# carrenD/Medical-Cross-Modality-Domain-Adaptation

Measured on AMD Instinct MI355X. Metric: training slices/sec (256x256x3, B=16/GPU) joint segmenter+GAN step (1 dis update on B MR + B CT, clip, 1 gen update on B CT), higher is better.
Workload: dtype f32; 1 GPU; BASELINE configs[3]: train_gan.py --phase train-gan joint step, B=16/GPU per domain, f32, dropout .75, mask critic on; global_batch=16, per_gpu_batch=16, parallelism=dp1, step_capture=False

## Files before the change

medical-cross-modality-domain-adaptation_amd/csrc/conv_common.h:

```cpp
#pragma once
#include "pnp_common.h"

namespace pnpconv {

constexpr int BK = 32;
constexpr int NTHREADS = 256;
#ifndef PNP_CONV_ABLATE
#define PNP_CONV_ABLATE 0
#endif
constexpr int kAblate = PNP_CONV_ABLATE;

struct ConvArgs {
    const float* x;
    const float* w;
    float* y;
    int N, H, W, C, K, R, S, OH, OW, stride, dil, pad_t, pad_l, pad_mode;
    int ups;
    int M;
    int Kred;
    int OHW;
    int nblk_m, nblk_n;
    int gn;
    int nsplit, chunks_per_split;
    long long split_stride;
// ... 302 lines not shown
int launch_x3_direct(const ConvArgs& a, int kind, bool flip_transpose, void* ws, size_t ws_bytes, hipStream_t st);
bool wino_chosen(const pnp_conv_geom* g);
int wino_tile(const pnp_conv_geom* g);
size_t wino_workspace_bytes(const pnp_conv_geom* g);
int wino_stats_parts(const pnp_conv_geom* g);
int launch_wino(const ConvArgs& a, int kind, bool flip_transpose, void* ws, size_t ws_bytes, hipStream_t st);
bool wino_wgrad_chosen(const pnp_conv_geom* g);
int wino_wgrad_tile(const pnp_conv_geom* g);
size_t wino_wgrad_workspace_bytes(const pnp_conv_geom* g);
int launch_wino_wgrad(const ConvArgs& a, float* dw, int accumulate, void* ws, size_t ws_bytes, hipStream_t st);
#ifndef PNP_X3_SW
#define PNP_X3_SW 32
#endif
constexpr int X3_SW = PNP_X3_SW;
static_assert(X3_SW == 16 || X3_SW == 32, "stage width");
bool wino_x3_dims_ok(int T, int C, int K);
int launch_wino_gemm_x3(const unsigned short* V3, const unsigned short* U3, float* Mm, int T, int C, int K, int npos, int sym, int gn, int xcd,
                        int nsplit, int stages_per_split, hipStream_t st);
inline double conv_flops(const ConvArgs& a) { return 2.0 * (double)a.M * a.K * a.Kred; }
inline double conv_bytes(const ConvArgs& a) {
    return 4.0 * ((double)a.N * a.H * a.W * a.C + (double)a.M * a.K + (double)a.Kred * a.K);
}
inline int prof_class(int kind) { return kind == 0 ? PNP_PROF_CONV_FWD : PNP_PROF_CONV_DGRAD; }

}
```

medical-cross-modality-domain-adaptation_amd/csrc/conv_wino.hip:

```cpp
#include <atomic>
#include <map>
#include <mutex>
#include "conv_common.h"
#include "conv_mma.h"

using namespace pnpconv;

namespace {

constexpr int NT = 256;

__device__ __forceinline__ f32x4 ld4(const float* p) { return *reinterpret_cast<const f32x4*>(p); }
__device__ __forceinline__ void st4(float* p, f32x4 v) { *reinterpret_cast<f32x4*>(p) = v; }

typedef __bf16 bf16x4 __attribute__((ext_vector_type(4)));
__device__ __forceinline__ void split3(float v, __bf16& hi, __bf16& mid, __bf16& lo) {
    hi = (__bf16)v;
    const float r = v - (float)hi;
    mid = (__bf16)r;
    lo = (__bf16)(r - (float)mid);
}
__device__ __forceinline__ void st4x3(__bf16* p, size_t pstride, f32x4 v) {
    bf16x4 h, m, l;
#pragma unroll
    for (int e = 0; e < 4; ++e) {
        __bf16 a, b, c;
        split3(v[e], a, b, c);
        h[e] = a; m[e] = b; l[e] = c;
    }
    *reinterpret_cast<bf16x4*>(p) = h;
    *reinterpret_cast<bf16x4*>(p + pstride) = m;
    *reinterpret_cast<bf16x4*>(p + 2 * pstride) = l;
}

struct WinoGeom {
    int N, Hi, Wi, Ho, Wo, dil, ps, Hsi, Wsi, Hso, Wso, th, tw, T;
    int m;
};

template <typename V>
__device__ __forceinline__ void w4_bt(const V& d0, const V& d1, const V& d2, const V& d3, const V& d4, const V& d5, V* o) {
    o[0] = (d0 + d4) + (1.5f * (d3 - d1) - 2.f * d2);
    o[1] = (d4 - d1) + (0.5f * d2 + 2.5f * d3);
    o[2] = (d4 + d1) + (0.5f * d3 - 2.5f * d2);
    o[3] = (d4 - d2) + 2.f * (d3 - d1);
    o[4] = (d4 - d2) + 0.5f * (d1 - d3);
    o[5] = (d1 + d5) + (1.5f * (d4 - d2) - 2.f * d3);
}
// ... 69 lines not shown
        f32x4 d[P][P];
#pragma unroll
        for (int p = 0; p < P; ++p) {
            const int u = M * ti - a.g.ps + p;
            const bool uok = (unsigned)u < (unsigned)a.g.Hsi;
#pragma unroll
            for (int q = 0; q < P; ++q) {
                const int v = M * tj - a.g.ps + q;
                const bool ok = uok & ((unsigned)v < (unsigned)a.g.Wsi);
                const unsigned off = (unsigned)(((n * a.g.Hi + pa + a.g.dil * u) * a.g.Wi + pb + a.g.dil * v) * a.C + c) * 4u;
                d[p][q] = bload4(rx, ok ? off : OOB);
            }
        }
        f32x4 r[P][P];
        float* out = a.V + (size_t)t * a.C + c;
        __bf16* out3 = reinterpret_cast<__bf16*>(a.V) + ((size_t)(c / X3_SW) * 3 * a.g.T + t) * X3_SW + (c % X3_SW);
        auto put = [&](int pos, f32x4 v) {
            if constexpr (X3) st4x3(out3 + (size_t)pos * 3 * plane, (size_t)a.g.T * X3_SW, v);
            else st4(out + (size_t)pos * plane, v);
        };
        if constexpr (M == 2) {
#pragma unroll
            for (int q = 0; q < 4; ++q) {
                r[0][q] = d[0][q] - d[2][q];
                r[1][q] = d[1][q] + d[2][q];
                r[2][q] = d[2][q] - d[1][q];
                r[3][q] = d[1][q] - d[3][q];
            }
#pragma unroll
            for (int p = 0; p < 4; ++p) {
                put(4 * p + 0, r[p][0] - r[p][2]);
                put(4 * p + 1, r[p][1] + r[p][2]);
                put(4 * p + 2, r[p][2] - r[p][1]);
                put(4 * p + 3, r[p][1] - r[p][3]);
            }
// ... 568 lines not shown
            f32x4 c6[6];
            w4_a(y[0][q], y[1][q], y[2][q], y[3][q], c6);
#pragma unroll
            for (int p = 0; p < 6; ++p) z[p][q] = c6[p];
        }
#pragma unroll
        for (int p = 0; p < 6; ++p) {
            f32x4 o[6];
            w4_a(z[p][0], z[p][1], z[p][2], z[p][3], o);
#pragma unroll
            for (int q = 0; q < 6; ++q) v[6 * p + q] = o[q];
        }
    }
}
template <int NP, int PG>
__device__ __forceinline__ void emit_t(const f32x4 (&v)[NP], float (*tile)[32][34], __bf16* __restrict__ out, size_t pos_stride, int tblk, int rows, int ch0,
                                       int tid) {
    const int c4 = tid & 7, tl = tid >> 3;
    const int cl = tid >> 3, tq = tid & 7;
#pragma unroll
    for (int r0 = 0; r0 < NP; r0 += PG) {
#pragma unroll
        for (int p = 0; p < PG; ++p)
#pragma unroll
            for (int e = 0; e < 4; ++e) tile[p][c4 * 4 + e][tl] = v[r0 + p][e];
        __syncthreads();
        if (ch0 + cl < rows) {
#pragma unroll
            for (int p = 0; p < PG; ++p) {
                const float* src = &tile[p][cl][4 * tq];
                const f32x4 w = {src[0], src[1], src[2], src[3]};
                const int tg = tblk * 32 + 4 * tq;
                st4x3(out + (size_t)(r0 + p) * pos_stride + ((size_t)(tg / X3_SW) * 3 * rows + ch0 + cl) * X3_SW + (tg % X3_SW), (size_t)rows * X3_SW, w);
            }
        }
        __syncthreads();
    }
}
struct WinoTArgs {
    const float* src;
    __bf16* out;
    WinoGeom g;
    int rows;
    unsigned src_bytes;
    int ntb;
};
template <int M>
__global__ void __launch_bounds__(NT) wino_in_t_kernel(WinoTArgs a) {
    constexpr int P = M + 2, NP = P * P, PG = M == 4 ? 12 : 8;
    __shared__ float tile[PG][32][34];
    const int tid = threadIdx.x, c4 = tid & 7, tl = tid >> 3;
    const int t = blockIdx.x * 32 + tl, c = blockIdx.y * 32 + c4 * 4;
    const bool tok = t < a.g.T;
    const __amdgpu_buffer_rsrc_t rx = make_rsrc(a.src, a.src_bytes);
    int n, pa, pb, ti, tj;
    tile_of(a.g, tok ? t : 0, n, pa, pb, ti, tj);
    f32x4 d[P][P];
#pragma unroll
    for (int p = 0; p < P; ++p) {
        const int u = M * ti - a.g.ps + p;
        const bool uok = tok & ((unsigned)u < (unsigned)a.g.Hsi);
#pragma unroll
        for (int q = 0; q < P; ++q) {
            const int v_ = M * tj - a.g.ps + q;
            const bool ok = uok & ((unsigned)v_ < (unsigned)a.g.Wsi);
            const unsigned off = (unsigned)(((n * a.g.Hi + pa + a.g.dil * u) * a.g.Wi + pb + a.g.dil * v_) * a.rows + c) * 4u;
            d[p][q] = bload4(rx, ok ? off : OOB);
        }
    }
    f32x4 v[NP];
    bt_2d<M>(d, v);
    emit_t<NP, PG>(v, tile, a.out, (size_t)a.ntb * 3 * a.rows * 32, (int)blockIdx.x, a.rows, (int)blockIdx.y * 32, tid);
}
template <int M>
__global__ void __launch_bounds__(NT) wino_dy_t_kernel(WinoTArgs a) {
    constexpr int P = M + 2, NP = P * P, PG = M == 4 ? 12 : 8;
    __shared__ float tile[PG][32][34];
    const int tid = threadIdx.x, c4 = tid & 7, tl = tid >> 3;
    const int t = blockIdx.x * 32 + tl, k = blockIdx.y * 32 + c4 * 4;
    const bool tok = t < a.g.T && k < a.rows;
    int n, pa, pb, ti, tj;
    tile_of(a.g, t < a.g.T ? t : 0, n, pa, pb, ti, tj);
    f32x4 y[M][M];
#pragma unroll
    for (int p = 0; p < M; ++p)
#pragma unroll
        for (int q = 0; q < M; ++q) {
            const int u = M * ti + p, v_ = M * tj + q;
            const f32x4 zero = {0, 0, 0, 0};
            y[p][q] = (tok && u < a.g.Hso && v_ < a.g.Wso) ? ld4(a.src + ((size_t)(n * a.g.Ho + pa + a.g.dil * u) * a.g.Wo + pb + a.g.dil * v_) * a.rows + k) : zero;
        }
    f32x4 v[NP];
    a_2d<M>(y, v);
    emit_t<NP, PG>(v, tile, a.out, (size_t)a.ntb * 3 * a.rows * 32, (int)blockIdx.x, a.rows, (int)blockIdx.y * 32, tid);
}

struct WinoWgradGemmArgs {
    const float* V;
    const float* Y;
    float* S;
    int T, C, K;
    int nblk_m, nblk_n, nsplit, chunks_per_split, xcd_swizzle;
    int npos;
};

template <int BM, int BN, int WM, int WN, int TILE>
__global__ void __launch_bounds__(NTHREADS, 2) wino_wgrad_gemm_kernel(WinoWgradGemmArgs g) {
    constexpr int TM = BM / WM / 32, TN = BN / WN / 32;
    constexpr int LDA = BM + 4, LDB = BN + 4;
// ... 379 lines not shown

int wino_stats_parts(const pnp_conv_geom* g) {
    if (x3d_chosen(g)) return x3d_stats_parts(g);
    const int m = plan_tile(g, false);
    const WinoGeom w = make_wgeom(g, m ? m : 2);
    int tpb, nblk;
    out_plan(w.T, g->K, &tpb, &nblk);
    return nblk;
}

template <int M>
static int launch_wino_m(const ConvArgs& a, int kind, bool flip_transpose, void* ws, size_t ws_bytes, hipStream_t st) {
    constexpr int NP = (M + 2) * (M + 2);
    const WinoGeom w = make_wgeom(a.N, a.H, a.W, a.OH, a.OW, a.dil, a.pad_t, M);
    const bool x3 = use_x3(w.T, a.C, a.K);
    const size_t eb = x3 ? 6 : 4;
    const size_t ub = al256((size_t)NP * a.C * a.K * eb), vb = al256((size_t)NP * w.T * a.C * eb), mb = al256((size_t)NP * w.T * a.K * 4);
    static const int xcd_mode = env_int("PNP_WINO_XCD", 2);
    const bool xcd = a.xcd_swizzle && xcd_mode;
    GemmPlan plan = gemm_plan(w.T, a.C, a.K, NP, xcd);
    if (x3) { plan.s = 1; plan.px_bytes = 0; }
    if (!ws || ws_bytes < ub + vb + mb + plan.px_bytes) {
        pnp_set_error("launch_wino: workspace too small (%zu < %zu)", ws_bytes, ub + vb + mb + plan.px_bytes);
        return PNP_EWORKSPACE;
    }
    PNP_REQUIRE(a.y_h == nullptr && a.o_s == 0 && a.ups == 1, "launch_wino: unsupported epilogue");
    bool run_filter;
    float* U = filter_slot(a.w, flip_transpose ? 1 : 0, M, a.C, a.K, x3 ? 1 : 0, (size_t)NP * a.C * a.K * eb, (float*)ws, st, &run_filter);
    float* V = (float*)((char*)ws + ub);
    float* Mm = (float*)((char*)ws + ub + vb);
    float* Px = (float*)((char*)ws + ub + vb + mb);
// ... 2 lines not shown
        dim3 grid((unsigned)pnp_cdiv(a.K, 32), (unsigned)pnp_cdiv(a.C, 32));
        PnpProfScope ps(cls, st, 0.0, (36.0 + eb * NP) * a.C * a.K, "wino_filter_kernel<%s, %d, %s>", flip_transpose ? "true" : "false", M, x3 ? "true" : "false");
        if (x3) {
            if (flip_transpose) hipLaunchKernelGGL((wino_filter_kernel<true, M, true>), grid, dim3(NT), 0, st, a.w, U, a.C, a.K);
            else hipLaunchKernelGGL((wino_filter_kernel<false, M, true>), grid, dim3(NT), 0, st, a.w, U, a.C, a.K);
        } else if (flip_transpose) hipLaunchKernelGGL((wino_filter_kernel<true, M, false>), grid, dim3(NT), 0, st, a.w, U, a.C, a.K);
        else hipLaunchKernelGGL((wino_filter_kernel<false, M, false>), grid, dim3(NT), 0, st, a.w, U, a.C, a.K);
        PNP_CHECK_LAUNCH("wino_filter_kernel");
    }
    {
        WinoInArgs ia{};
        ia.x = a.x; ia.V = V; ia.g = w; ia.C = a.C; ia.x_bytes = a.x_bytes; ia.xcd = a.xcd_swizzle ? env_xcd_in() : 0;
        const size_t nvec = (size_t)w.T * (a.C / 4);
        long long nb = (long long)((nvec + NT - 1) / NT);
        if (nb > 65536) nb = 65536;
        PnpProfScope ps(cls, st, 0.0, 4.0 * (double)a.N * a.H * a.W * a.C + (double)eb * NP * w.T * a.C, "wino_in_kernel<%d, %s>", M, x3 ? "true" : "false");
        if (x3) hipLaunchKernelGGL((wino_in_kernel<M, true>), dim3((unsigned)nb), dim3(NT), 0, st, ia);
        else hipLaunchKernelGGL((wino_in_kernel<M, false>), dim3((unsigned)nb), dim3(NT), 0, st, ia);
        PNP_CHECK_LAUNCH("wino_in_kernel");
    }
    if (x3) {
        static const int wino_gn3 = env_int("PNP_WINO_GN", -1);
        const int rc = launch_wino_gemm_x3((const unsigned short*)V, (const unsigned short*)U, Mm, w.T, a.C, a.K, NP, (M == 4 ? 2 : 0) + (kind != 0), wino_gn3 >= 0 ? wino_gn3 : a.gn,
                                           xcd ? 1 : 0, 1, a.C / 32, st);
        if (rc != PNP_OK) return rc;
    } else {
        WinoGemmArgs ga{};
        ga.V = V; ga.U = U; ga.Mm = Mm; ga.T = w.T; ga.C = a.C; ga.K = a.K;
        const bool narrow = a.K <= 64;
        ga.nblk_m = pnp_cdiv(w.T, 128); ga.nblk_n = pnp_cdiv(a.K, narrow ? 64 : 128);
        static const int wino_gn = env_int("PNP_WINO_GN", -1);
        ga.gn = wino_gn >= 0 ? wino_gn : a.gn; ga.xcd_swizzle = xcd ? 2 : 0;
        ga.npos = NP;
        ga.whole = ((double)NP * w.T * a.C * 4.0 < 2147483648.0 && (double)NP * a.C * a.K * 4.0 < 2147483648.0) ? 1 : 0;
        ga.tail_F = plan.F; ga.tail_R = plan.R; ga.tail_s = plan.s; ga.Px = Px;
        dim3 grid((unsigned)plan.grid);
        const double fl = 2.0 * NP * (double)w.T * a.C * a.K;
        const double by = 4.0 * NP * ((double)w.T * a.C + (double)a.C * a.K + (double)w.T * a.K);
// ... 81 lines not shown
}

template <int M>
static int launch_wino_wgrad_m(const ConvArgs& a, float* dw, int accumulate, void* ws, size_t ws_bytes, hipStream_t st) {
    constexpr int NP = (M + 2) * (M + 2);
    const WinoGeom w = make_wgeom(a.N, a.H, a.W, a.OH, a.OW, a.dil, a.pad_t, M);
    if (use_x3_wgrad(w.T, a.C, a.K)) {
        int sps;
        const int ns = wgrad_split_x3(w.T, a.C, a.K, NP, &sps);
        const int tp = x3_tp(w.T), ntb = tp / 32;
        const size_t vb = al256((size_t)NP * tp * a.C * 6), yb = al256((size_t)NP * tp * a.K * 6), sb = al256((size_t)ns * NP * a.C * a.K * 4);
        if (!ws || ws_bytes < vb + yb + sb) {
            pnp_set_error("launch_wino_wgrad: workspace too small (%zu < %zu)", ws_bytes, vb + yb + sb);
            return PNP_EWORKSPACE;
        }
        __bf16* V3 = (__bf16*)ws;
        __bf16* Y3 = (__bf16*)((char*)ws + vb);
        float* S = (float*)((char*)ws + vb + yb);
        {
            WinoTArgs ta{};
            ta.src = a.x; ta.out = V3; ta.g = w; ta.rows = a.C; ta.src_bytes = a.x_bytes; ta.ntb = ntb;
            PnpProfScope ps(PNP_PROF_CONV_WGRAD, st, 0.0, 4.0 * (double)a.N * a.H * a.W * a.C + 6.0 * NP * tp * a.C, "wino_in_t_kernel<%d>", M);
            hipLaunchKernelGGL(wino_in_t_kernel<M>, dim3((unsigned)ntb, (unsigned)(a.C / 32)), dim3(NT), 0, st, ta);
            PNP_CHECK_LAUNCH("wino_in_t_kernel");
        }
        {
            WinoTArgs ta{};
            ta.src = a.w; ta.out = Y3; ta.g = w; ta.rows = a.K; ta.src_bytes = 0; ta.ntb = ntb;
            PnpProfScope ps(PNP_PROF_CONV_WGRAD, st, 0.0, 4.0 * (double)a.M * a.K + 6.0 * NP * tp * a.K, "wino_dy_t_kernel<%d>", M);
            hipLaunchKernelGGL(wino_dy_t_kernel<M>, dim3((unsigned)ntb, (unsigned)pnp_cdiv(a.K, 32)), dim3(NT), 0, st, ta);
            PNP_CHECK_LAUNCH("wino_dy_t_kernel");
        }
        const int rc = launch_wino_gemm_x3((const unsigned short*)V3, (const unsigned short*)Y3, S, a.C, tp, a.K, NP, M == 4 ? 5 : 4, 0, a.xcd_swizzle ? 1 : 0, ns, sps, st);
        if (rc != PNP_OK) return rc;
        int ns_out = ns;
        if (ns > 2 && (size_t)a.C * (a.K / 4) < (size_t)NT * 512) {
            const size_t nv = (size_t)NP * a.C * (a.K / 4);
            PnpProfScope ps(PNP_PROF_CONV_WGRAD, st, 0.0, 4.0 * ((double)ns + 1.0) * NP * a.C * a.K, "wino_splitsum_kernel");
            hipLaunchKernelGGL(wino_splitsum_kernel, dim3((unsigned)((nv + NT - 1) / NT)), dim3(NT), 0, st, S, nv, ns);
            PNP_CHECK_LAUNCH("wino_splitsum_kernel");
            ns_out = 1;
        }
        const size_t nvec = (size_t)a.C * (a.K / 4);
        PnpProfScope ps(PNP_PROF_CONV_WGRAD, st, 0.0, 4.0 * ((double)ns_out * NP + 9.0 * (1 + (accumulate != 0))) * a.C * a.K, "wino_wgrad_out_kernel<%d>", M);
        hipLaunchKernelGGL(wino_wgrad_out_kernel<M>, dim3((unsigned)((nvec + NT - 1) / NT)), dim3(NT), 0, st, (const float*)S, dw, a.C, a.K, ns_out, accumulate);
        PNP_CHECK_LAUNCH("wino_wgrad_out_kernel");
        return PNP_OK;
    }
// ... 120 lines not shown
```

medical-cross-modality-domain-adaptation_amd/csrc/conv_wino_x3.hip:

```cpp
#include <type_traits>
#include "conv_common.h"

using namespace pnpconv;

namespace {

typedef __bf16 bf16x8 __attribute__((ext_vector_type(8)));
typedef __attribute__((address_space(3))) void lds_void;
#ifndef PNP_X3_AUX
#define PNP_X3_AUX 0
#endif

template <int N>
__device__ __forceinline__ void wait_vm() {
    asm volatile("s_waitcnt vmcnt(%0)" ::"n"(N) : "memory");
}
__device__ __forceinline__ void wait_lgkm0() { asm volatile("s_waitcnt lgkmcnt(0)" ::: "memory"); }
__device__ __forceinline__ void dma16(__amdgpu_buffer_rsrc_t r, lds_void* dst, unsigned voff, int soff) {
#if defined(__HIP_DEVICE_COMPILE__)
    __builtin_amdgcn_raw_ptr_buffer_load_lds(r, dst, 16, voff, soff, 0, PNP_X3_AUX);
#endif
}

struct X3Args {
    const unsigned short* V;
    const unsigned short* U;
    float* Mm;
    int T, C, K, npos;
    int nblk_m, nblk_n, gn, xcd;
    int nsplit, spz;
};

template <int SW>
__device__ __forceinline__ int swz(int row) {
    return SW == 32 ? ((row >> 2) & 3) : ((row >> 3) & 1);
}

#ifndef PNP_X3_NL
#define PNP_X3_NL 4
#endif
template <int BM, int BN, int KIND>
__global__ void __launch_bounds__(64 * (BM / 32 + PNP_X3_NL), (BM / 32 + PNP_X3_NL) / 4) wino_gemm_x3_kernel(X3Args g) {
    constexpr int SW = X3_SW;
    constexpr int NCW = BM / 32;
    constexpr int kTermA[6] = {2, 1, 0, 1, 0, 0}, kTermB[6] = {0, 1, 2, 0, 1, 0};
    constexpr int NL = PNP_X3_NL;
    constexpr int ROWB = 2 * SW;
    constexpr int LPR = ROWB / 16;
    constexpr int RPI = 64 / LPR;
    constexpr int KS = SW / 16;
    constexpr int NPA = 3 * BM / RPI, NPB = 3 * BN / RPI, NP = NPA + NPB;
    constexpr int LPS = (NP + NL - 1) / NL;
    constexpr int TM = 2, TN = BN / 2 / 32;
    constexpr int APL = BM * ROWB, BPL = BN * ROWB;
    constexpr int STG = 3 * (APL + BPL);
    constexpr int NBUF = (147456 / STG) < 8 ? (147456 / STG) : 8;
    constexpr int SPC = 64 / SW;
    static_assert(NBUF >= 2 && (NBUF - 2) * LPS < 64, "vmcnt is a 6-bit counter");
    __shared__ __attribute__((aligned(256))) unsigned char lds[NBUF * STG];

    const int t = threadIdx.x;
    const int lane = t & 63;
    const int wave = __builtin_amdgcn_readfirstlane(t >> 6);
    const int nblk = g.nblk_m * g.nblk_n;
    const int nitems = nblk * g.npos * g.nsplit;
    int base = 0, cnt = nitems, first = (int)blockIdx.x, step = (int)gridDim.x;
    if (g.xcd) {
        const int NX = 8, x = (int)blockIdx.x % NX, q = nitems / NX, r = nitems % NX;
        base = (x < r) ? x * (q + 1) : r * (q + 1) + (x - r) * q;
        cnt = q + (x < r ? 1 : 0);
        first = (int)blockIdx.x / NX;
        step = ((int)gridDim.x - x + NX - 1) / NX;
    }
// ... 7 lines not shown
        tile_coords(item - pz * nblk, g.nblk_m, g.nblk_n, g.gn, mt, nt);
        m0 = mt * BM;
        n0 = nt * BN;
        s0 = z * g.spz;
        nst = min(g.spz, nstage_all - s0);
    };
    int gstages = 0;
    for (int it = first; it < cnt; it += step) {
        int pos, z, m0, n0, s0, nst;
        decode(base + it, pos, z, m0, n0, s0, nst);
        gstages += nst;
    }

    if (wave >= NCW) {
        const int lw = wave - NCW;
        const int lrow = lane / LPR, lchk = lane % LPR;
        const size_t planeV = (size_t)3 * g.T * g.C, planeU = (size_t)3 * g.K * g.C;
        const __amdgpu_buffer_rsrc_t rv = make_rsrc(reinterpret_cast<const float*>(g.V), (unsigned)(planeV * g.npos * 2));
        const __amdgpu_buffer_rsrc_t ru = make_rsrc(reinterpret_cast<const float*>(g.U), (unsigned)(planeU * g.npos * 2));
        const int sstrideV = 3 * g.T * ROWB, sstrideU = 3 * g.K * ROWB;
        unsigned pvo[LPS];
        int pdst[LPS];
        bool pisa[LPS];
#pragma unroll
        for (int i = 0; i < LPS; ++i) {
            int q = i * NL + lw;
            if (q >= NP) q -= NL;
            pisa[i] = q < NPA;
            const int qq = pisa[i] ? q : q - NPA, rows = pisa[i] ? BM : BN;
            pdst[i] = (pisa[i] ? 0 : 3 * APL) + (qq / (rows / RPI)) * (pisa[i] ? APL : BPL) + (qq % (rows / RPI)) * (RPI * ROWB);
        }
        int c_it = first, c_j = 0, c_nst = 0, c_s0 = 0;
        auto setup = [&](int it) {
            int pos, z, m0, n0;
            decode(base + it, pos, z, m0, n0, c_s0, c_nst);
            const unsigned pv = (unsigned)(pos * planeV * 2), pu = (unsigned)(pos * planeU * 2);
#pragma unroll
            for (int i = 0; i < LPS; ++i) {
                int q = i * NL + lw;
                if (q >= NP) q -= NL;
                const bool isa = q < NPA;
                const int qq = isa ? q : q - NPA, rows = isa ? BM : BN, lim = isa ? g.T : g.K;
                const int plane = qq / (rows / RPI), rb = qq % (rows / RPI);
                const int r = rb * RPI + lrow, m = (isa ? m0 : n0) + r;
                pvo[i] = (m < lim) ? (isa ? pv : pu) + (unsigned)((plane * lim + m) * ROWB + ((lchk ^ swz<SW>(r)) << 4)) : OOB2;
            }
        };
        setup(c_it);
        auto issue_next = [&](int buf) {
            unsigned char* bp = lds + buf * STG;
            const int cc = c_s0 + c_j;
#pragma unroll
            for (int i = 0; i < LPS; ++i) {
                if (pisa[i]) dma16(rv, (lds_void*)(bp + pdst[i]), pvo[i], cc * sstrideV);
                else dma16(ru, (lds_void*)(bp + pdst[i]), pvo[i], cc * sstrideU);
            }
            if (c_j + 1 < c_nst) {
                ++c_j;
            } else if (c_it + step < cnt) {
                c_it += step;
                c_j = 0;
                setup(c_it);
            }
        };
#pragma unroll
        for (int b_ = 0; b_ < NBUF - 1; ++b_) issue_next(b_);
        int nb = NBUF - 1;
        for (int gsi = 0; gsi < gstages; ++gsi) {
            wait_vm<(NBUF - 2) * LPS>();
            __builtin_amdgcn_s_barrier();
            issue_next(nb);
            nb = nb == NBUF - 1 ? 0 : nb + 1;
        }
        wait_vm<0>();
        return;
    }
    const int wm0 = (wave >> 1) * 64, wn0 = (wave & 1) * (BN / 2);
    const int l31 = lane & 31, h = lane >> 5;
    int foff[KS];
#pragma unroll
    for (int ks = 0; ks < KS; ++ks) foff[ks] = l31 * ROWB + (((2 * ks + h) ^ swz<SW>(l31)) << 4);

    Acc<TM, TN> cur, total;
    int buf = 0;
    auto stage = [&](auto fc) {
        constexpr bool first_ = decltype(fc)::value;
        wait_lgkm0();
        __builtin_amdgcn_s_barrier();
        asm volatile("" ::: "memory");
// ... 45 lines not shown
#pragma unroll
                for (int tn = 0; tn < TN; ++tn) total.v[tm][tn] += cur.v[tm][tn];
        }
        conv_epilogue<TM, TN>(e, total, g.Mm + ((size_t)z * g.npos + pos) * g.T * g.K, m0, n0, wm0, wn0, lane, 0);
    }
}

}

namespace pnpconv {

bool wino_x3_dims_ok(int T, int C, int K) {
    return (C % 64) == 0 && 36.0 * T * C * 6.0 < 2147483648.0 && 36.0 * K * C * 6.0 < 2147483648.0;
}

int launch_wino_gemm_x3(const unsigned short* V3, const unsigned short* U3, float* Mm, int T, int C, int K, int npos, int sym, int gn, int xcd,
                        int nsplit, int stages_per_split, hipStream_t st) {
    PNP_REQUIRE(wino_x3_dims_ok(T, C, K), "launch_wino_gemm_x3: operands too large for one buffer descriptor per transform point");
    PNP_REQUIRE(sym >= 0 && sym < 6, "launch_wino_gemm_x3: bad symbol index");
    stages_per_split *= 32 / X3_SW;
    PNP_REQUIRE(nsplit >= 1 && (stages_per_split % (64 / X3_SW)) == 0 && (long long)nsplit * stages_per_split >= C / X3_SW &&
                    (long long)(nsplit - 1) * stages_per_split < C / X3_SW,
                "launch_wino_gemm_x3: bad reduction split");
    X3Args g{};
    g.V = V3; g.U = U3; g.Mm = Mm; g.T = T; g.C = C; g.K = K; g.npos = npos;
    const bool narrow = K <= 64;
    static const int bm_force = getenv("PNP_X3_BM") ? atoi(getenv("PNP_X3_BM")) : 0;
    const bool tall = !narrow && bm_force == 256 && T >= 256;
    g.nblk_m = pnp_cdiv(T, tall ? 256 : 128); g.nblk_n = pnp_cdiv(K, narrow ? 64 : 128);
    g.gn = gn; g.xcd = xcd ? 1 : 0;
    g.nsplit = nsplit; g.spz = stages_per_split;
    const long long nitems = (long long)g.nblk_m * g.nblk_n * npos * nsplit;
    static const int persist = getenv("PNP_X3_PERSIST") ? atoi(getenv("PNP_X3_PERSIST")) : 1;
    const dim3 grid((unsigned)((persist && nitems > 256) ? 256 : nitems));
    const double fl = 6.0 * 2.0 * npos * (double)T * C * K;
    const double by = (double)npos * (6.0 * ((double)T * C + (double)C * K) + 4.0 * (double)nsplit * T * K);
    PnpProfScope ps(sym >= 4 ? PNP_PROF_CONV_WGRAD : prof_class(sym & 1), st, fl, by, "wino_gemm_x3_kernel<%d, %d, %d>", tall ? 256 : 128, narrow ? 64 : 128, sym);
#define PNP_X3_LAUNCH(BN_, SYM_) hipLaunchKernelGGL((wino_gemm_x3_kernel<128, BN_, SYM_>), grid, dim3(64 * (4 + PNP_X3_NL)), 0, st, g)
#define PNP_X3_LAUNCH_TALL(SYM_) hipLaunchKernelGGL((wino_gemm_x3_kernel<256, 128, SYM_>), grid, dim3(64 * (8 + PNP_X3_NL)), 0, st, g)
    if (tall) {
        switch (sym) {
            case 0: PNP_X3_LAUNCH_TALL(0); break;
            case 1: PNP_X3_LAUNCH_TALL(1); break;
            case 2: PNP_X3_LAUNCH_TALL(2); break;
            case 3: PNP_X3_LAUNCH_TALL(3); break;
            case 4: PNP_X3_LAUNCH_TALL(4); break;
            default: PNP_X3_LAUNCH_TALL(5); break;
        }
    } else if (narrow) {
        switch (sym) {
            case 0: PNP_X3_LAUNCH(64, 0); break;
// ... 24 lines not shown
```

medical-cross-modality-domain-adaptation_amd/csrc/conv_x3_direct.hip:

```cpp
#include <atomic>
#include <cstdlib>
#include "conv_common.h"

using namespace pnpconv;

namespace {

typedef __bf16 bf16x8 __attribute__((ext_vector_type(8)));
typedef __bf16 bf16x4 __attribute__((ext_vector_type(4)));
typedef __attribute__((address_space(3))) void lds_void;

constexpr int TH = 16, TW = 16, PH = TH + 2, PW = TW + 2, NPX = PH * PW;
constexpr int ROWB = 64;
constexpr int PLANE_P = NPX * ROWB;
constexpr int PATCH = 3 * PLANE_P;
constexpr int NF = 3;
constexpr int LDS_BYTES = 2 * PATCH + NF * 3 * 64 * ROWB;
constexpr int NPL = 192;
constexpr int NPI = (NPX * 8 + NPL - 1) / NPL;

__device__ __forceinline__ int swz(int row) { return (row >> 2) & 3; }
__device__ __forceinline__ void wait_lgkm0() { asm volatile("s_waitcnt lgkmcnt(0)" ::: "memory"); }
__device__ __forceinline__ void wait_vm0() { asm volatile("s_waitcnt vmcnt(0)" ::: "memory"); }
template <int N>
// ... 98 lines not shown
                if (ok) v = *reinterpret_cast<const f32x4*>(a.x + (((size_t)n * a.H + ih) * a.W + iw) * a.C + hsel * 32 + j * 4);
                st[i] = v;
            }
        };
        auto store = [&](int slot, int i0, int i1) {
            unsigned char* pb = patch0 + (slot & 1) * PATCH;
#pragma unroll
            for (int i = 0; i < NPI; ++i) {
                if (i < i0 || i >= i1) continue;
                const int e = pl + i * NPL;
                if (e >= NPX * 8) continue;
                const int q = e >> 3, j = e & 7;
                bf16x4 hi, mi, lo;
#pragma unroll
                for (int c = 0; c < 4; ++c) {
                    const float v = st[i][c];
                    const __bf16 h = (__bf16)v;
                    const float r1 = v - (float)h;
                    const __bf16 m = (__bf16)r1;
                    const float r2 = r1 - (float)m;
                    hi[c] = h; mi[c] = m; lo[c] = (__bf16)r2;
                }
                const int off = q * ROWB + (((j >> 1) ^ swz(q)) << 4) + (j & 1) * 8;
                *reinterpret_cast<bf16x4*>(pb + off) = hi;
                *reinterpret_cast<bf16x4*>(pb + PLANE_P + off) = mi;
                *reinterpret_cast<bf16x4*>(pb + 2 * PLANE_P + off) = lo;
            }
        };
        const int nslots = myitems * NH;
        load(0);
        wait_vm0();
        store(0, 0, NPI);
        for (int g = 0; g < gstages; ++g) {
            const int slot = g / 9, j = g - slot * 9;
            if (j == 0) wait_lgkm0();
            __builtin_amdgcn_s_barrier();
// ... 142 lines not shown
    }
}

template <bool FLIP>
__global__ void __launch_bounds__(256) x3d_filter_kernel(const float* __restrict__ w, unsigned short* __restrict__ w3, int C, int K, int KW) {
    const int NH = C >> 5, KB = K / KW;
    const int total = KB * NH * 9 * KW * 32;
    const int e = blockIdx.x * 256 + threadIdx.x;
    if (e >= total) return;
    const int i = e & 31, o = (e >> 5) % KW;
    int r = (e >> 5) / KW;
    const int tap = r % 9; r /= 9;
    const int hf = r % NH, kb = r / NH;
    const int ic = hf * 32 + i, oc = kb * KW + o;
    const float v = FLIP ? w[((size_t)(8 - tap) * K + oc) * C + ic] : w[((size_t)tap * C + ic) * K + oc];
    const __bf16 b0 = (__bf16)v;
    const float r1 = v - (float)b0;
    const __bf16 b1 = (__bf16)r1;
    const float r2 = r1 - (float)b1;
    const __bf16 b2 = (__bf16)r2;
    const size_t base = ((((size_t)kb * NH + hf) * 9 + tap) * 3) * ((size_t)KW * 32) + (size_t)o * 32 + i;
    w3[base] = __builtin_bit_cast(unsigned short, b0);
    w3[base + (size_t)KW * 32] = __builtin_bit_cast(unsigned short, b1);
    w3[base + 2 * (size_t)KW * 32] = __builtin_bit_cast(unsigned short, b2);
}

std::atomic<int> g_x3d_mode{-1};

int x3d_mode() {
    int m = g_x3d_mode.load(std::memory_order_relaxed);
    if (m < 0) {
        m = getenv("PNP_X3_DIRECT") ? atoi(getenv("PNP_X3_DIRECT")) : 1;
        g_x3d_mode.store(m, std::memory_order_relaxed);
    }
    return m;
// ... 73 lines not shown
```

Baseline: 275.0 slices/s.

## Stage Winograd GEMM operands as f32 and split to bf16x3 in-kernel

The Winograd input and wgrad transform kernels now write plain f32 tiles instead of pre-split hi/mid/lo bf16 planes. The x3 GEMM loader waves load f32 through registers and perform the three-way bf16 split while writing into LDS. The forward/dgrad filter operand stays pre-split, and the direct LDS DMA loads are replaced. The aim is to cut transform-output bytes (4 instead of 6 per element) and global traffic, at the cost of extra ALU work, register pressure in the loader waves, and losing asynchronous DMA to LDS.

Result: no change. 276.4 slices/s, median of 6 (+0.5%).

```diff
diff --git a/medical-cross-modality-domain-adaptation_amd/csrc/conv_common.h b/medical-cross-modality-domain-adaptation_amd/csrc/conv_common.h
--- a/medical-cross-modality-domain-adaptation_amd/csrc/conv_common.h
+++ b/medical-cross-modality-domain-adaptation_amd/csrc/conv_common.h
@@ -340,8 +340,14 @@
 #endif
 constexpr int X3_SW = PNP_X3_SW;
 static_assert(X3_SW == 16 || X3_SW == 32, "stage width");
+__device__ __forceinline__ void split3(float v, __bf16& hi, __bf16& mid, __bf16& lo) {
+    hi = (__bf16)v;
+    const float r = v - (float)hi;
+    mid = (__bf16)r;
+    lo = (__bf16)(r - (float)mid);
+}
 bool wino_x3_dims_ok(int T, int C, int K);
-int launch_wino_gemm_x3(const unsigned short* V3, const unsigned short* U3, float* Mm, int T, int C, int K, int npos, int sym, int gn, int xcd,
+int launch_wino_gemm_x3(const float* V, const void* U, float* Mm, int T, int C, int K, int npos, int sym, int gn, int xcd,
                         int nsplit, int stages_per_split, hipStream_t st);
 inline double conv_flops(const ConvArgs& a) { return 2.0 * (double)a.M * a.K * a.Kred; }
 inline double conv_bytes(const ConvArgs& a) {
diff --git a/medical-cross-modality-domain-adaptation_amd/csrc/conv_wino.hip b/medical-cross-modality-domain-adaptation_amd/csrc/conv_wino.hip
--- a/medical-cross-modality-domain-adaptation_amd/csrc/conv_wino.hip
+++ b/medical-cross-modality-domain-adaptation_amd/csrc/conv_wino.hip
@@ -13,25 +13,6 @@
 __device__ __forceinline__ f32x4 ld4(const float* p) { return *reinterpret_cast<const f32x4*>(p); }
 __device__ __forceinline__ void st4(float* p, f32x4 v) { *reinterpret_cast<f32x4*>(p) = v; }
 
-typedef __bf16 bf16x4 __attribute__((ext_vector_type(4)));
-__device__ __forceinline__ void split3(float v, __bf16& hi, __bf16& mid, __bf16& lo) {
-    hi = (__bf16)v;
-    const float r = v - (float)hi;
-    mid = (__bf16)r;
-    lo = (__bf16)(r - (float)mid);
-}
-__device__ __forceinline__ void st4x3(__bf16* p, size_t pstride, f32x4 v) {
-    bf16x4 h, m, l;
-#pragma unroll
-    for (int e = 0; e < 4; ++e) {
-        __bf16 a, b, c;
-        split3(v[e], a, b, c);
-        h[e] = a; m[e] = b; l[e] = c;
-    }
-    *reinterpret_cast<bf16x4*>(p) = h;
-    *reinterpret_cast<bf16x4*>(p + pstride) = m;
-    *reinterpret_cast<bf16x4*>(p + 2 * pstride) = l;
-}
 
 struct WinoGeom {
     int N, Hi, Wi, Ho, Wo, dil, ps, Hsi, Wsi, Hso, Wso, th, tw, T;
@@ -131,11 +112,8 @@
         }
         f32x4 r[P][P];
         float* out = a.V + (size_t)t * a.C + c;
-        __bf16* out3 = reinterpret_cast<__bf16*>(a.V) + ((size_t)(c / X3_SW) * 3 * a.g.T + t) * X3_SW + (c % X3_SW);
-        auto put = [&](int pos, f32x4 v) {
-            if constexpr (X3) st4x3(out3 + (size_t)pos * 3 * plane, (size_t)a.g.T * X3_SW, v);
-            else st4(out + (size_t)pos * plane, v);
-        };
+        float* out3 = a.V + ((size_t)(c / X3_SW) * a.g.T + t) * X3_SW + (c % X3_SW);
+        auto put = [&](int pos, f32x4 v) { st4((X3 ? out3 : out) + (size_t)pos * plane, v); };
         if constexpr (M == 2) {
 #pragma unroll
             for (int q = 0; q < 4; ++q) {
@@ -734,7 +712,7 @@
     }
 }
 template <int NP, int PG>
-__device__ __forceinline__ void emit_t(const f32x4 (&v)[NP], float (*tile)[32][34], __bf16* __restrict__ out, size_t pos_stride, int tblk, int rows, int ch0,
+__device__ __forceinline__ void emit_t(const f32x4 (&v)[NP], float (*tile)[32][34], float* __restrict__ out, size_t pos_stride, int tblk, int rows, int ch0,
                                        int tid) {
     const int c4 = tid & 7, tl = tid >> 3;
     const int cl = tid >> 3, tq = tid & 7;
@@ -751,7 +729,7 @@
                 const float* src = &tile[p][cl][4 * tq];
                 const f32x4 w = {src[0], src[1], src[2], src[3]};
                 const int tg = tblk * 32 + 4 * tq;
-                st4x3(out + (size_t)(r0 + p) * pos_stride + ((size_t)(tg / X3_SW) * 3 * rows + ch0 + cl) * X3_SW + (tg % X3_SW), (size_t)rows * X3_SW, w);
+                st4(out + (size_t)(r0 + p) * pos_stride + ((size_t)(tg / X3_SW) * rows + ch0 + cl) * X3_SW + (tg % X3_SW), w);
             }
         }
         __syncthreads();
@@ -759,7 +737,7 @@
 }
 struct WinoTArgs {
     const float* src;
-    __bf16* out;
+    float* out;
     WinoGeom g;
     int rows;
     unsigned src_bytes;
@@ -790,7 +768,7 @@
     }
     f32x4 v[NP];
     bt_2d<M>(d, v);
-    emit_t<NP, PG>(v, tile, a.out, (size_t)a.ntb * 3 * a.rows * 32, (int)blockIdx.x, a.rows, (int)blockIdx.y * 32, tid);
+    emit_t<NP, PG>(v, tile, a.out, (size_t)a.ntb * a.rows * 32, (int)blockIdx.x, a.rows, (int)blockIdx.y * 32, tid);
 }
 template <int M>
 __global__ void __launch_bounds__(NT) wino_dy_t_kernel(WinoTArgs a) {
@@ -812,7 +790,7 @@
         }
     f32x4 v[NP];
     a_2d<M>(y, v);
-    emit_t<NP, PG>(v, tile, a.out, (size_t)a.ntb * 3 * a.rows * 32, (int)blockIdx.x, a.rows, (int)blockIdx.y * 32, tid);
+    emit_t<NP, PG>(v, tile, a.out, (size_t)a.ntb * a.rows * 32, (int)blockIdx.x, a.rows, (int)blockIdx.y * 32, tid);
 }
 
 struct WinoWgradGemmArgs {
@@ -1222,7 +1200,7 @@
     constexpr int NP = (M + 2) * (M + 2);
     const WinoGeom w = make_wgeom(a.N, a.H, a.W, a.OH, a.OW, a.dil, a.pad_t, M);
     const bool x3 = use_x3(w.T, a.C, a.K);
-    const size_t eb = x3 ? 6 : 4;
+    const size_t eb = x3 ? 6 : 4, tb = 4;
     const size_t ub = al256((size_t)NP * a.C * a.K * eb), vb = al256((size_t)NP * w.T * a.C * eb), mb = al256((size_t)NP * w.T * a.K * 4);
     static const int xcd_mode = env_int("PNP_WINO_XCD", 2);
     const bool xcd = a.xcd_swizzle && xcd_mode;
@@ -1255,14 +1233,14 @@
         const size_t nvec = (size_t)w.T * (a.C / 4);
         long long nb = (long long)((nvec + NT - 1) / NT);
         if (nb > 65536) nb = 65536;
-        PnpProfScope ps(cls, st, 0.0, 4.0 * (double)a.N * a.H * a.W * a.C + (double)eb * NP * w.T * a.C, "wino_in_kernel<%d, %s>", M, x3 ? "true" : "false");
+        PnpProfScope ps(cls, st, 0.0, 4.0 * (double)a.N * a.H * a.W * a.C + (double)tb * NP * w.T * a.C, "wino_in_kernel<%d, %s>", M, x3 ? "true" : "false");
         if (x3) hipLaunchKernelGGL((wino_in_kernel<M, true>), dim3((unsigned)nb), dim3(NT), 0, st, ia);
         else hipLaunchKernelGGL((wino_in_kernel<M, false>), dim3((unsigned)nb), dim3(NT), 0, st, ia);
         PNP_CHECK_LAUNCH("wino_in_kernel");
     }
     if (x3) {
         static const int wino_gn3 = env_int("PNP_WINO_GN", -1);
-        const int rc = launch_wino_gemm_x3((const unsigned short*)V, (const unsigned short*)U, Mm, w.T, a.C, a.K, NP, (M == 4 ? 2 : 0) + (kind != 0), wino_gn3 >= 0 ? wino_gn3 : a.gn,
+        const int rc = launch_wino_gemm_x3(V, U, Mm, w.T, a.C, a.K, NP, (M == 4 ? 2 : 0) + (kind != 0), wino_gn3 >= 0 ? wino_gn3 : a.gn,
                                            xcd ? 1 : 0, 1, a.C / 32, st);
         if (rc != PNP_OK) return rc;
     } else {
@@ -1374,24 +1352,24 @@
             pnp_set_error("launch_wino_wgrad: workspace too small (%zu < %zu)", ws_bytes, vb + yb + sb);
             return PNP_EWORKSPACE;
         }
-        __bf16* V3 = (__bf16*)ws;
-        __bf16* Y3 = (__bf16*)((char*)ws + vb);
+        float* Vt = (float*)ws;
+        float* Yt = (float*)((char*)ws + vb);
         float* S = (float*)((char*)ws + vb + yb);
         {
             WinoTArgs ta{};
-            ta.src = a.x; ta.out = V3; ta.g = w; ta.rows = a.C; ta.src_bytes = a.x_bytes; ta.ntb = ntb;
-            PnpProfScope ps(PNP_PROF_CONV_WGRAD, st, 0.0, 4.0 * (double)a.N * a.H * a.W * a.C + 6.0 * NP * tp * a.C, "wino_in_t_kernel<%d>", M);
+            ta.src = a.x; ta.out = Vt; ta.g = w; ta.rows = a.C; ta.src_bytes = a.x_bytes; ta.ntb = ntb;
+            PnpProfScope ps(PNP_PROF_CONV_WGRAD, st, 0.0, 4.0 * (double)a.N * a.H * a.W * a.C + 4.0 * NP * tp * a.C, "wino_in_t_kernel<%d>", M);
             hipLaunchKernelGGL(wino_in_t_kernel<M>, dim3((unsigned)ntb, (unsigned)(a.C / 32)), dim3(NT), 0, st, ta);
             PNP_CHECK_LAUNCH("wino_in_t_kernel");
         }
         {
             WinoTArgs ta{};
-            ta.src = a.w; ta.out = Y3; ta.g = w; ta.rows = a.K; ta.src_bytes = 0; ta.ntb = ntb;
-            PnpProfScope ps(PNP_PROF_CONV_WGRAD, st, 0.0, 4.0 * (double)a.M * a.K + 6.0 * NP * tp * a.K, "wino_dy_t_kernel<%d>", M);
+            ta.src = a.w; ta.out = Yt; ta.g = w; ta.rows = a.K; ta.src_bytes = 0; ta.ntb = ntb;
+            PnpProfScope ps(PNP_PROF_CONV_WGRAD, st, 0.0, 4.0 * (double)a.M * a.K + 4.0 * NP * tp * a.K, "wino_dy_t_kernel<%d>", M);
             hipLaunchKernelGGL(wino_dy_t_kernel<M>, dim3((unsigned)ntb, (unsigned)pnp_cdiv(a.K, 32)), dim3(NT), 0, st, ta);
             PNP_CHECK_LAUNCH("wino_dy_t_kernel");
         }
-        const int rc = launch_wino_gemm_x3((const unsigned short*)V3, (const unsigned short*)Y3, S, a.C, tp, a.K, NP, M == 4 ? 5 : 4, 0, a.xcd_swizzle ? 1 : 0, ns, sps, st);
+        const int rc = launch_wino_gemm_x3(Vt, Yt, S, a.C, tp, a.K, NP, M == 4 ? 5 : 4, 0, a.xcd_swizzle ? 1 : 0, ns, sps, st);
         if (rc != PNP_OK) return rc;
         int ns_out = ns;
         if (ns > 2 && (size_t)a.C * (a.K / 4) < (size_t)NT * 512) {
diff --git a/medical-cross-modality-domain-adaptation_amd/csrc/conv_wino_x3.hip b/medical-cross-modality-domain-adaptation_amd/csrc/conv_wino_x3.hip
--- a/medical-cross-modality-domain-adaptation_amd/csrc/conv_wino_x3.hip
+++ b/medical-cross-modality-domain-adaptation_amd/csrc/conv_wino_x3.hip
@@ -6,25 +6,13 @@
 namespace {
 
 typedef __bf16 bf16x8 __attribute__((ext_vector_type(8)));
-typedef __attribute__((address_space(3))) void lds_void;
-#ifndef PNP_X3_AUX
-#define PNP_X3_AUX 0
-#endif
-
-template <int N>
-__device__ __forceinline__ void wait_vm() {
-    asm volatile("s_waitcnt vmcnt(%0)" ::"n"(N) : "memory");
-}
+typedef __bf16 bf16x4 __attribute__((ext_vector_type(4)));
+
 __device__ __forceinline__ void wait_lgkm0() { asm volatile("s_waitcnt lgkmcnt(0)" ::: "memory"); }
-__device__ __forceinline__ void dma16(__amdgpu_buffer_rsrc_t r, lds_void* dst, unsigned voff, int soff) {
-#if defined(__HIP_DEVICE_COMPILE__)
-    __builtin_amdgcn_raw_ptr_buffer_load_lds(r, dst, 16, voff, soff, 0, PNP_X3_AUX);
-#endif
-}
 
 struct X3Args {
-    const unsigned short* V;
-    const unsigned short* U;
+    const float* V;
+    const void* U;
     float* Mm;
     int T, C, K, npos;
     int nblk_m, nblk_n, gn, xcd;
@@ -46,17 +34,20 @@
     constexpr int kTermA[6] = {2, 1, 0, 1, 0, 0}, kTermB[6] = {0, 1, 2, 0, 1, 0};
     constexpr int NL = PNP_X3_NL;
     constexpr int ROWB = 2 * SW;
-    constexpr int LPR = ROWB / 16;
-    constexpr int RPI = 64 / LPR;
+    constexpr int LPR = SW / 4;
+    constexpr int RPL = 64 / LPR;
     constexpr int KS = SW / 16;
-    constexpr int NPA = 3 * BM / RPI, NPB = 3 * BN / RPI, NP = NPA + NPB;
-    constexpr int LPS = (NP + NL - 1) / NL;
+    constexpr bool B3 = KIND < 4;
+    constexpr int RPP = 64 / (ROWB / 16);
+    constexpr int NPA = BM / RPL, NPB = B3 ? 3 * BN / RPP : BN / RPL;
+    static_assert(NPA % NL == 0, "every loader wave loads the same pieces of A");
+    constexpr int LPA = NPA / NL, LPS = LPA + (NPB + NL - 1) / NL;
     constexpr int TM = 2, TN = BN / 2 / 32;
     constexpr int APL = BM * ROWB, BPL = BN * ROWB;
     constexpr int STG = 3 * (APL + BPL);
     constexpr int NBUF = (147456 / STG) < 8 ? (147456 / STG) : 8;
     constexpr int SPC = 64 / SW;
-    static_assert(NBUF >= 2 && (NBUF - 2) * LPS < 64, "vmcnt is a 6-bit counter");
+    static_assert(NBUF >= 2, "stages in LDS");
     __shared__ __attribute__((aligned(256))) unsigned char lds[NBUF * STG];
 
     const int t = threadIdx.x;
@@ -94,47 +85,53 @@
 
     if (wave >= NCW) {
         const int lw = wave - NCW;
-        const int lrow = lane / LPR, lchk = lane % LPR;
-        const size_t planeV = (size_t)3 * g.T * g.C, planeU = (size_t)3 * g.K * g.C;
-        const __amdgpu_buffer_rsrc_t rv = make_rsrc(reinterpret_cast<const float*>(g.V), (unsigned)(planeV * g.npos * 2));
-        const __amdgpu_buffer_rsrc_t ru = make_rsrc(reinterpret_cast<const float*>(g.U), (unsigned)(planeU * g.npos * 2));
-        const int sstrideV = 3 * g.T * ROWB, sstrideU = 3 * g.K * ROWB;
+        const int lrow = lane / LPR, lc = lane % LPR;
+        const int prow = lane / (ROWB / 16), pchk = lane % (ROWB / 16);
+        const size_t planeV = (size_t)g.T * g.C, planeU = (size_t)(B3 ? 3 : 1) * g.K * g.C;
+        const __amdgpu_buffer_rsrc_t rv = make_rsrc(g.V, (unsigned)(planeV * g.npos * 4));
+        const __amdgpu_buffer_rsrc_t ru = make_rsrc(reinterpret_cast<const float*>(g.U), (unsigned)(planeU * g.npos * (B3 ? 2 : 4)));
+        const int sstrideV = g.T * SW * 4, sstrideU = g.K * SW * (B3 ? 6 : 4);
+        auto bpiece = [&](int i) {
+            int q = (i - LPA) * NL + lw;
+            if (q >= NPB) q -= NL;
+            return q;
+        };
+        int pdst[LPS];
+#pragma unroll
+        for (int i = 0; i < LPS; ++i) {
+            if (i < LPA || !B3) {
+                const int r = (i < LPA ? i * NL + lw : bpiece(i)) * RPL + lrow;
+                pdst[i] = (i < LPA ? 0 : 3 * APL) + r * ROWB + (((lc >> 1) ^ swz<SW>(r)) << 4) + (lc & 1) * 8;
+            } else {
+                const int q = bpiece(i);
+                pdst[i] = 3 * APL + (q / (BN / RPP)) * BPL + ((q % (BN / RPP)) * RPP + prow) * ROWB + (pchk << 4);
+            }
+        }
         unsigned pvo[LPS];
-        int pdst[LPS];
-        bool pisa[LPS];
-#pragma unroll
-        for (int i = 0; i < LPS; ++i) {
-            int q = i * NL + lw;
-            if (q >= NP) q -= NL;
-            pisa[i] = q < NPA;
-            const int qq = pisa[i] ? q : q - NPA, rows = pisa[i] ? BM : BN;
-            pdst[i] = (pisa[i] ? 0 : 3 * APL) + (qq / (rows / RPI)) * (pisa[i] ? APL : BPL) + (qq % (rows / RPI)) * (RPI * ROWB);
-        }
         int c_it = first, c_j = 0, c_nst = 0, c_s0 = 0;
         auto setup = [&](int it) {
             int pos, z, m0, n0;
             decode(base + it, pos, z, m0, n0, c_s0, c_nst);
-            const unsigned pv = (unsigned)(pos * planeV * 2), pu = (unsigned)(pos * planeU * 2);
+            const unsigned pv = (unsigned)(pos * planeV * 4), pu = (unsigned)(pos * planeU * (B3 ? 2 : 4));
 #pragma unroll
             for (int i = 0; i < LPS; ++i) {
-                int q = i * NL + lw;
-                if (q >= NP) q -= NL;
-                const bool isa = q < NPA;
-                const int qq = isa ? q : q - NPA, rows = isa ? BM : BN, lim = isa ? g.T : g.K;
-                const int plane = qq / (rows / RPI), rb = qq % (rows / RPI);
-                const int r = rb * RPI + lrow, m = (isa ? m0 : n0) + r;
-                pvo[i] = (m < lim) ? (isa ? pv : pu) + (unsigned)((plane * lim + m) * ROWB + ((lchk ^ swz<SW>(r)) << 4)) : OOB2;
+                if (i < LPA) {
+                    const int m = m0 + i * NL * RPL + lw * RPL + lrow;
+                    pvo[i] = (m < g.T) ? pv + (unsigned)((m * SW + lc * 4) * 4) : OOB2;
+                } else if (!B3) {
+                    const int m = n0 + bpiece(i) * RPL + lrow;
+                    pvo[i] = (m < g.K) ? pu + (unsigned)((m * SW + lc * 4) * 4) : OOB2;
+                } else {
+                    const int q = bpiece(i), r = (q % (BN / RPP)) * RPP + prow, m = n0 + r;
+                    pvo[i] = (m < g.K) ? pu + (unsigned)(((q / (BN / RPP)) * g.K + m) * ROWB + ((pchk ^ swz<SW>(r)) << 4)) : OOB2;
+                }
             }
         };
         setup(c_it);
-        auto issue_next = [&](int buf) {
-            unsigned char* bp = lds + buf * STG;
+        auto load_next = [&](f32x4 (&rg)[LPS]) {
             const int cc = c_s0 + c_j;
 #pragma unroll
-            for (int i = 0; i < LPS; ++i) {
-                if (pisa[i]) dma16(rv, (lds_void*)(bp + pdst[i]), pvo[i], cc * sstrideV);
-                else dma16(ru, (lds_void*)(bp + pdst[i]), pvo[i], cc * sstrideU);
-            }
+            for (int i = 0; i < LPS; ++i) rg[i] = i < LPA ? bload4s(rv, pvo[i], cc * sstrideV) : bload4s(ru, pvo[i], cc * sstrideU);
             if (c_j + 1 < c_nst) {
                 ++c_j;
             } else if (c_it + step < cnt) {
@@ -143,16 +140,50 @@
                 setup(c_it);
             }
         };
-#pragma unroll
-        for (int b_ = 0; b_ < NBUF - 1; ++b_) issue_next(b_);
-        int nb = NBUF - 1;
-        for (int gsi = 0; gsi < gstages; ++gsi) {
-            wait_vm<(NBUF - 2) * LPS>();
+        auto put = [&](const f32x4 (&rg)[LPS], int buf) {
+            unsigned char* bp = lds + buf * STG;
+#pragma unroll
+            for (int i = 0; i < LPS; ++i) {
+                if (B3 && i >= LPA) {
+                    *reinterpret_cast<f32x4*>(bp + pdst[i]) = rg[i];
+                    continue;
+                }
+                bf16x4 hi, mid, lo;
+#pragma unroll
+                for (int e = 0; e < 4; ++e) {
+                    __bf16 a, b, c;
+                    split3(rg[i][e], a, b, c);
+                    hi[e] = a; mid[e] = b; lo[e] = c;
+                }
+                const int pl = i < LPA ? APL : BPL;
+                *reinterpret_cast<bf16x4*>(bp + pdst[i]) = hi;
+                *reinterpret_cast<bf16x4*>(bp + pdst[i] + pl) = mid;
+                *reinterpret_cast<bf16x4*>(bp + pdst[i] + 2 * pl) = lo;
+            }
+        };
+        f32x4 ra[LPS], rb[LPS];
+#pragma unroll
+        for (int b_ = 0; b_ < NBUF - 1; ++b_) {
+            load_next(ra);
+            put(ra, b_);
+        }
+        load_next(ra);
+        load_next(rb);
+        auto step_ = [&](f32x4 (&rg)[LPS], int gsi, int nb) {
+            wait_lgkm0();
             __builtin_amdgcn_s_barrier();
-            issue_next(nb);
+            asm volatile("" ::: "memory");
+            if (gsi + NBUF - 1 < gstages) put(rg, nb);
+            load_next(rg);
+        };
+        int nb = NBUF - 1, gsi = 0;
+        for (; gsi + 1 < gstages; gsi += 2) {
+            step_(ra, gsi, nb);
             nb = nb == NBUF - 1 ? 0 : nb + 1;
-        }
-        wait_vm<0>();
+            step_(rb, gsi + 1, nb);
+            nb = nb == NBUF - 1 ? 0 : nb + 1;
+        }
+        if (gsi < gstages) step_(ra, gsi, nb);
         return;
     }
     const int wm0 = (wave >> 1) * 64, wn0 = (wave & 1) * (BN / 2);
@@ -228,7 +259,7 @@
     return (C % 64) == 0 && 36.0 * T * C * 6.0 < 2147483648.0 && 36.0 * K * C * 6.0 < 2147483648.0;
 }
 
-int launch_wino_gemm_x3(const unsigned short* V3, const unsigned short* U3, float* Mm, int T, int C, int K, int npos, int sym, int gn, int xcd,
+int launch_wino_gemm_x3(const float* V, const void* U, float* Mm, int T, int C, int K, int npos, int sym, int gn, int xcd,
                         int nsplit, int stages_per_split, hipStream_t st) {
     PNP_REQUIRE(wino_x3_dims_ok(T, C, K), "launch_wino_gemm_x3: operands too large for one buffer descriptor per transform point");
     PNP_REQUIRE(sym >= 0 && sym < 6, "launch_wino_gemm_x3: bad symbol index");
@@ -237,7 +268,7 @@
                     (long long)(nsplit - 1) * stages_per_split < C / X3_SW,
                 "launch_wino_gemm_x3: bad reduction split");
     X3Args g{};
-    g.V = V3; g.U = U3; g.Mm = Mm; g.T = T; g.C = C; g.K = K; g.npos = npos;
+    g.V = V; g.U = U; g.Mm = Mm; g.T = T; g.C = C; g.K = K; g.npos = npos;
     const bool narrow = K <= 64;
     static const int bm_force = getenv("PNP_X3_BM") ? atoi(getenv("PNP_X3_BM")) : 0;
     const bool tall = !narrow && bm_force == 256 && T >= 256;
@@ -248,7 +279,7 @@
     static const int persist = getenv("PNP_X3_PERSIST") ? atoi(getenv("PNP_X3_PERSIST")) : 1;
     const dim3 grid((unsigned)((persist && nitems > 256) ? 256 : nitems));
     const double fl = 6.0 * 2.0 * npos * (double)T * C * K;
-    const double by = (double)npos * (6.0 * ((double)T * C + (double)C * K) + 4.0 * (double)nsplit * T * K);
+    const double by = (double)npos * (4.0 * (double)T * C + (sym >= 4 ? 4.0 : 6.0) * (double)C * K + 4.0 * (double)nsplit * T * K);
     PnpProfScope ps(sym >= 4 ? PNP_PROF_CONV_WGRAD : prof_class(sym & 1), st, fl, by, "wino_gemm_x3_kernel<%d, %d, %d>", tall ? 256 : 128, narrow ? 64 : 128, sym);
 #define PNP_X3_LAUNCH(BN_, SYM_) hipLaunchKernelGGL((wino_gemm_x3_kernel<128, BN_, SYM_>), grid, dim3(64 * (4 + PNP_X3_NL)), 0, st, g)
 #define PNP_X3_LAUNCH_TALL(SYM_) hipLaunchKernelGGL((wino_gemm_x3_kernel<256, 128, SYM_>), grid, dim3(64 * (8 + PNP_X3_NL)), 0, st, g)
diff --git a/medical-cross-modality-domain-adaptation_amd/csrc/conv_x3_direct.hip b/medical-cross-modality-domain-adaptation_amd/csrc/conv_x3_direct.hip
--- a/medical-cross-modality-domain-adaptation_amd/csrc/conv_x3_direct.hip
+++ b/medical-cross-modality-domain-adaptation_amd/csrc/conv_x3_direct.hip
@@ -136,12 +136,9 @@
                 bf16x4 hi, mi, lo;
 #pragma unroll
                 for (int c = 0; c < 4; ++c) {
-                    const float v = st[i][c];
-                    const __bf16 h = (__bf16)v;
-                    const float r1 = v - (float)h;
-                    const __bf16 m = (__bf16)r1;
-                    const float r2 = r1 - (float)m;
-                    hi[c] = h; mi[c] = m; lo[c] = (__bf16)r2;
+                    __bf16 h, m, l;
+                    split3(st[i][c], h, m, l);
+                    hi[c] = h; mi[c] = m; lo[c] = l;
                 }
                 const int off = q * ROWB + (((j >> 1) ^ swz(q)) << 4) + (j & 1) * 8;
                 *reinterpret_cast<bf16x4*>(pb + off) = hi;
@@ -314,11 +311,8 @@
     const int hf = r % NH, kb = r / NH;
     const int ic = hf * 32 + i, oc = kb * KW + o;
     const float v = FLIP ? w[((size_t)(8 - tap) * K + oc) * C + ic] : w[((size_t)tap * C + ic) * K + oc];
-    const __bf16 b0 = (__bf16)v;
-    const float r1 = v - (float)b0;
-    const __bf16 b1 = (__bf16)r1;
-    const float r2 = r1 - (float)b1;
-    const __bf16 b2 = (__bf16)r2;
+    __bf16 b0, b1, b2;
+    split3(v, b0, b1, b2);
     const size_t base = ((((size_t)kb * NH + hf) * 9 + tap) * 3) * ((size_t)KW * 32) + (size_t)o * 32 + i;
     w3[base] = __builtin_bit_cast(unsigned short, b0);
     w3[base + (size_t)KW * 32] = __builtin_bit_cast(unsigned short, b1);
```
